# theori-io/nrsc5

Measured on NVIDIA H100. Metric: cu8 I/Q Msamples/s, higher is better.
Workload: dtype u8/int16/f32

## Files before the change

nrsc5_b200/csrc/front.cuh:

```cuda
#pragma once
#include "pids_crc.cuh"
#include "common.cuh"
#include "fft.cuh"
#include "viterbi_pack.cuh"

namespace nb {

constexpr int FRONT_THREADS = 1024;
constexpr int TEAMS = FRONT_THREADS / 128;
constexpr int MAXREF = 15;
constexpr int IN_BYTES = 4 * NSYM + 28 + 16 + 16;
constexpr int IN_STRIDE = 8704;
constexpr int ACQ_TILE = 4096;

__device__ int g_dbg;

__constant__ int c_compat_mode[64];
__constant__ unsigned c_pn80[3];
__constant__ short c_bp_tap[32];

__device__ __forceinline__ float2 cmulf(float2 a, float2 b)
{
    return make_float2(a.x * b.x - a.y * b.y, a.x * b.y + a.y * b.x);
}
__device__ __forceinline__ float2 cexp_j(float a)
{
    float s, c;
    sincosf(a, &s, &c);
    return make_float2(c, s);
}

__device__ __forceinline__ int partitions_per_band(int psmi)
{
    switch (c_compat_mode[psmi & 63]) {
    case 2: return 11;
    case 3: return 12;
    case 5: case 6: case 11: return 14;
    default: return 10;
    }
}

__device__ void set_state(const DevPtrs &p, const EngineDims &d, int s, int ns)
{
    StreamState &st = p.st[s];
    if (st.state == ns) return;
    if (st.state == ST_FINE) log_reserve(p, d, s, REC_LOST_SYNC, 0);
    if (ns == ST_FINE) {
        float fo = (float)(((double)st.prev_angle - 2 * M_PI * st.cfo) * 744187.5 / (2 * M_PI * NFFT));
        uint8_t *w = log_reserve(p, d, s, REC_SYNC, 8);
        if (w) {
            reinterpret_cast<float *>(w)[0] = fo;
            reinterpret_cast<int *>(w)[1] = st.psmi;
        }
    }
    st.state = ns;
}

constexpr int DEMOD_RUN = 17;
constexpr int TEAM_SMEM = IN_STRIDE + NSYM * (int)sizeof(short2);
struct DemodSmem {
    float2 buf[TEAMS][TEAM_SMEM / sizeof(float2)];
    float2 symphase[TEAMS];
};
static_assert(FFT_SMEM_ELEMS * sizeof(float2) <= TEAM_SMEM && TEAM_SMEM % 16 == 0, "a team's FFT buffer");
static_assert(DEMOD_RUN * FFT_THREADS >= NSYM && DEMOD_RUN % 2 == 1, "a symbol's runs");
struct PrepSmem {
    uint32_t words[ACQ_TILE + 40];
    short2 ytile[ACQ_TILE + 32];
    float2 sums[NSYM];
    float red_mag[FRONT_THREADS];
    int red_idx[FRONT_THREADS];
    float2 red_v[FRONT_THREADS];
};
constexpr int ACQ1_RUN = 3;
constexpr int ACQ1_WORDS = (NSYM + 38 + 3 + 3) / 4 * 4;
static_assert(ACQ1_RUN * FRONT_THREADS >= NSYM + 31 && ACQ1_RUN % 2 == 1, "a tile's runs");
struct Acq1Smem {
    uint32_t words[2][ACQ1_WORDS];
    short2 ytile[NSYM + 32];
    float2 ring[2][NSYM];
    float2 sums[NSYM];
    float2 shape[NCP];
    float red_mag[FRONT_THREADS];
    int red_idx[FRONT_THREADS];
    float2 red_v[FRONT_THREADS];
};
struct PidsSmem {
    int8_t vit[PIDS_LEN * 3];
    uint2 dec[PIDS_LEN + 64];
};
constexpr int ZS = 32;
static_assert(2 * MAXREF <= 32, "a reference slot fits the 5 bits of FrontSmem::ref_plan");
constexpr int EQ_LD = BLK + 1;
constexpr int EQ_MAXPART = 12;
constexpr int EQ_ROWS = 2 * EQ_MAXPART * (PW - 1);
struct SyncSmem {
    float phs[BLK][ZS];
    float2 eph[2 * MAXREF][BLK];
    float smag[2 * MAXREF];
    float cfq[2 * MAXREF];
    union {
        float2 eq[EQ_ROWS][EQ_LD];
        struct {
            int offs[76][22];
            int verdict[76];
            int winner;
        } srch;
    };
    float wred[FRONT_THREADS / 32][2];
    float fb_w[2][MAXREF], fb_xy[2][MAXREF + 1];
    float4 rowc[EQ_ROWS];
    int ref_ok[2 * MAXREF], ref_bc[2 * MAXREF], ref_psmi[2 * MAXREF];
    bool px_on[2];
    long long px_T[2];
    uint8_t *soft_w;
    int do_search;
};
struct FrontSmem {
    float2 tw[FFT_TW];
    float2 nco[NSYM];
    float2 zref[BLK][ZS];
    uint8_t ref_plan[128];
    union {
        DemodSmem demod;
        PrepSmem prep;
        Acq1Smem acq1;
        SyncSmem sync;
        PidsSmem pidsq[16];
    } u;
};

__device__ void pids_decode_warp(const DevPtrs &p, const EngineDims &d, int s, int e, PidsSmem &sm, int lane)
{
    const StreamState &st = p.st[s];
    const int bc = st.pids_bc[e];
    const int8_t *pmall = p.pm + (size_t)s * 16 * PM_BLOCK;
    const int8_t PMV[20] = { 10, 2, 18, 6, 14, 8, 16, 0, 12, 4, 11, 3, 19, 7, 15, 9, 17, 1, 13, 5 };
    for (int o = lane; o < PIDS_LEN * 3; o += 32) {
        int8_t v = 0;
        if (o % 6 != 5) {
            unsigned i = (unsigned)bc * 200 + (unsigned)(o - o / 6);
            unsigned part = (unsigned)PMV[i % 20];
            unsigned block = i / 200;
            unsigned k = (i / 20) % 10 + P1_ENC / 320;
            unsigned row = (k * 11) % 32, col = (k * 11 + k / 288) % 36;
            v = pmall[(block * 32 + row) * 720 + part * 36 + col];
        }
        sm.vit[o] = v;
    }
    __syncwarp();
    const int l = lane & 15;
    VitHalf<false> vh;
    vh.init(l);
    vitc_run<false>(vh, sm.vit, PIDS_LEN, PIDS_LEN + 64, 0, PIDS_LEN + 64, 0, sm.dec, lane < 16, l);
    __syncwarp();
    int v = (short)(vh.E & 0xffff), state = 2 * l;
    const int w1 = (short)(vh.O & 0xffff);
    if (w1 > v) { v = w1; state = 2 * l + 1; }
    int v2 = (short)(vh.E >> 16), idx2 = 2 * l + 32;
    const int w3 = (short)(vh.O >> 16);
    if (w3 > v2) { v2 = w3; idx2 = 2 * l + 33; }
    if (v2 > v) { v = v2; state = idx2; }
#pragma unroll
    for (int o = 8; o; o >>= 1) {
        const int ov = __shfl_xor_sync(0xffffffffu, v, o, 16), oi = __shfl_xor_sync(0xffffffffu, state, o, 16);
        if (ov > v || (ov == v && oi < state)) { v = ov; state = oi; }
    }
    if (lane == 0) {
        uint8_t pk[10];
        for (int i = 0; i < 10; i++) pk[i] = 0;
        for (int q = PIDS_LEN + 63; q >= 0; q--) {
            if (q >= 32 && q < 32 + PIDS_LEN) {
                const int i = q - 32;
// ... 4 lines not shown
        }
        if (st.pids_rec[e] != 0xffffffffu) {
            uint8_t *w = p.log + (size_t)s * d.log_cap + st.pids_rec[e];
            for (int i = 0; i < 10; i++) w[i] = pk[i];
            w[10] = (uint8_t)pids_crc12_ok(pk);
        }
    }
}

__device__ void front_pids_flush(const DevPtrs &p, const EngineDims &d, int s, PidsSmem *sm, int t)
{
    StreamState &st = p.st[s];
    const int n = st.pids_pending, warp = t >> 5;
    if (warp < n) pids_decode_warp(p, d, s, warp, sm[warp], t & 31);
    __syncthreads();
    if (t == 0) st.pids_pending = 0;
}

constexpr int ACQ_RUN = 5;
static_assert(ACQ_RUN * FRONT_THREADS >= ACQ_TILE + 31, "a tile's runs");
template <int RUN>
__device__ __forceinline__ void acq_tile_input(const EngineDims &d, const uint32_t *words, short2 *ytile, const StreamState &st,
                                               int i0, int L, int t)
{
    const int kb = i0 == 0 ? 31 : 0;
    if (t < kb) ytile[t] = make_short2(st.bp_hist[t][0], st.bp_hist[t][1]);
    const int n = L + 31 - kb;
    if (d.cs16) {
        for (int k = kb + t; k < L + 31; k += FRONT_THREADS) {
            const uint32_t w = words[k + 7];
            ytile[k] = make_short2((short)(w & 0xffff), (short)(w >> 16));
        }
    } else if (RUN * t < n) {
        const int k = kb + min(RUN * t, n - RUN);
        halfband_run<RUN>(words + k, ytile + k);
    }
}

__device__ __forceinline__ float2 acq_bandpass(const short2 *yy)
{
    short accr = 0, acci = 0;
#pragma unroll 5
    for (int k = 1; k < 16; k++) {
        const short2 a = yy[k], b = yy[32 - k];
        accr = (short)(accr + ((((int)a.x + (int)b.x) * c_bp_tap[k]) >> 15));
        acci = (short)(acci + ((((int)a.y + (int)b.y) * c_bp_tap[k]) >> 15));
    }
    const short2 c = yy[16];
    accr = (short)(accr + (((int)c.x * c_bp_tap[16]) >> 15));
    acci = (short)(acci + (((int)c.y * c_bp_tap[16]) >> 15));
    return make_float2(__fdiv_rn((float)accr, 32767.0f), __fdiv_rn((float)acci, -32767.0f));
}

__device__ __forceinline__ void fill_nco(const DevPtrs &p, float2 *nco, float theta, int t)
{
    for (int j = t; j < NSYM; j += FRONT_THREADS) {
        float2 e = cexp_j(theta * (float)j);
        if (j < NCP || j >= NFFT) {
            const float w = __ldg(&p.shape[j]);
            e = make_float2(e.x * w, e.y * w);
        }
        nco[j] = e;
    }
}

__device__ int front_prep_begin(const DevPtrs &p, const EngineDims &d, int s, int t)
{
    StreamState &st = p.st[s];
    __shared__ int sh_active;
    if (t == 0) {
        if (st.force_state >= 0) {
            set_state(p, d, s, st.force_state);
            st.force_state = -1;
        }
        const long long avail = *reinterpret_cast<volatile long long *>(&st.in_avail);
        int act = avail >= 2 * (st.start + NACQ);
        if (act && st.state == ST_FINE) {
            const int need = px_need_of(c_compat_mode[st.psmi & 63]);
            if (need & ~d.px_enabled) {
                atomicOr(&p.ctl->px_need, (unsigned)need);
                act = 0;
            }
        }
        st.active = act;
        sh_active = act ? (st.state == ST_FINE ? 1 : 2) : 0;
        if (act) atomicAdd(&p.ctl->progress, 1ull);
    }
    __syncthreads();
    const int mode = sh_active;
    __syncthreads();
    return mode;
}

__device__ void front_acq_tiles(const DevPtrs &p, const EngineDims &d, int s, PrepSmem &sm, int t, int rank, int nranks)
{
    StreamState &st = p.st[s];
    const uint8_t *iq = p.iq + (size_t)s * d.in_stride;
    float2 *tb = p.tbuf + (size_t)s * NACQ;
    const long long start = nranks > 1 ? __ldcg(&st.start) : st.start;
    const uint32_t *iqw = reinterpret_cast<const uint32_t *>(iq);
    for (int i0 = rank * ACQ_TILE; i0 < NACQ; i0 += nranks * ACQ_TILE) {
        const int L = min(ACQ_TILE, NACQ - i0);
        const long long w0 = start + i0 - 38;
        for (int v = t; v < L + 38; v += FRONT_THREADS) {
            const long long a = w0 + v;
            sm.words[v] = a >= 0 ? __ldcg(iqw + a) : (d.cs16 ? 0u : 0x7f7f7f7fu);
        }
        __syncthreads();
        acq_tile_input<ACQ_RUN>(d, sm.words, sm.ytile, st, i0, L, t);
        __syncthreads();
        for (int j = t; j < L; j += FRONT_THREADS) tb[i0 + j] = acq_bandpass(sm.ytile + j);
        if (i0 + L == NACQ && t < 31) {
            const short2 v = sm.ytile[L + t];
            st.bp_hist_next[t][0] = v.x;
            st.bp_hist_next[t][1] = v.y;
        }
        __syncthreads();
    }
}

__device__ void front_acq_corr(const DevPtrs &p, int s, int t, int rank, int nranks)
{
    const float2 *tb = p.tbuf + (size_t)s * NACQ;
    float2 *sums = p.acq_sums + (size_t)s * NSYM;
    const int lo = rank * NSYM / nranks, hi = (rank + 1) * NSYM / nranks;
    for (int i = lo + t; i < hi; i += FRONT_THREADS) {
        float2 acc = make_float2(0.f, 0.f);
        for (int j = 0; j < BLK; j++) {
            const float2 a = __ldcg(&tb[i + j * NSYM]), b = __ldcg(&tb[i + j * NSYM + NFFT]);
            float2 pr = cmulf(a, make_float2(b.x, -b.y));
            acc.x += pr.x;
            acc.y += pr.y;
        }
        sums[i] = acc;
    }
}

__device__ void front_prep_finish(const DevPtrs &p, const EngineDims &d, int s, PrepSmem &sm, float2 *nco, int t, int mode)
{
    StreamState &st = p.st[s];
    __shared__ int sh_samperr;
    __shared__ float sh_angle, sh_theta;
    const int state_in = st.state;
    if (mode == 2) {
        const float2 *gs = p.acq_sums + (size_t)s * NSYM;
        for (int i = t; i < NSYM; i += FRONT_THREADS) sm.sums[i] = __ldcg(&gs[i]);
        if (t < 31) {
            st.bp_hist[t][0] = __ldcg(&st.bp_hist_next[t][0]);
            st.bp_hist[t][1] = __ldcg(&st.bp_hist_next[t][1]);
        }
        __syncthreads();
        float best = -1.0f;
        int besti = 0;
        float2 bestv = make_float2(0.f, 0.f);
        for (int i = t; i < NSYM; i += FRONT_THREADS) {
            float2 v = make_float2(0.f, 0.f);
            for (int j = 0; j < NCP; j++) {
                int q = i + j;
                if (q >= NSYM) q -= NSYM;
                const float2 sv = sm.sums[q];
                const float a = __ldg(&p.shape[j]), b = __ldg(&p.shape[j + NFFT]);
                v.x += (sv.x * a) * b;
                v.y += (sv.y * a) * b;
            }
            const float mag = v.x * v.x + v.y * v.y;
            if (mag > best) { best = mag; besti = i; bestv = v; }
        }
        sm.red_mag[t] = best; sm.red_idx[t] = besti; sm.red_v[t] = bestv;
        __syncthreads();
        for (int o = FRONT_THREADS / 2; o; o >>= 1) {
            if (t < o) {
                const float m2 = sm.red_mag[t + o];
                const int i2 = sm.red_idx[t + o];
                if (m2 > sm.red_mag[t] || (m2 == sm.red_mag[t] && i2 < sm.red_idx[t])) {
                    sm.red_mag[t] = m2; sm.red_idx[t] = i2; sm.red_v[t] = sm.red_v[t + o];
                }
            }
            __syncthreads();
        }
        if (t == 0) {
            const float2 w = cmulf(sm.red_v[0], cexp_j(-st.prev_angle));
            const float angle_diff = atan2f(w.y, w.x);
            const float factor = (st.prev_angle != 0.0f) ? 0.25f : 1.0f;
            const float angle = st.prev_angle + (angle_diff * factor);
            st.prev_angle = angle;
            sh_angle = angle;
            sh_samperr = (sm.red_idx[0] + NSYM - 15) % NSYM;
            if (st.state == ST_NONE) st.state = ST_COARSE;
        }
    } else if (t == 0) {
        sh_samperr = NSYM / 2 + st.samperr;
        st.samperr = 0;
        const float angle = st.prev_angle + (-st.angle);
        st.angle = 0;
        st.prev_angle = angle;
        sh_angle = angle;
    }
    __syncthreads();

    const int samperr = sh_samperr;
    const int adj = NSYM / 2 - samperr;
    if (adj != 0) {
        float *cp = p.cphase + (size_t)s * NFFT;
        for (int i = t; i < SIDE; i += FRONT_THREADS) {
            const int bl = LB0 + i, bu = UB1 - i;
            cp[bl] = (float)((double)cp[bl] - (double)(adj * (bl - NFFT / 2) * 2) * M_PI / NFFT);
            cp[bu] = (float)((double)cp[bu] - (double)(adj * (bu - NFFT / 2) * 2) * M_PI / NFFT);
        }
    }
    if (t == 0) {
        float angle = sh_angle;
        angle = (float)((double)angle - 2 * M_PI * st.cfo);
        const float pre = (float)(-adj) * angle / (float)NFFT;
        const float2 ph = cmulf(st.phase, cexp_j(pre));
        const float theta = angle / (float)NFFT;
        st.phase0 = ph;
        st.theta = theta;
        sh_theta = theta;
        st.blk_samperr = samperr;
        st.blk_state_in = state_in;
        double sn, cs;
        sincos((double)theta * (double)(NSYM * BLK), &sn, &cs);
        const float2 pe = cmulf(ph, make_float2((float)cs, (float)sn));
        const float nrm = sqrtf(pe.x * pe.x + pe.y * pe.y);
        st.phase = make_float2(pe.x / nrm, pe.y / nrm);
        uint8_t *w = log_reserve(p, d, s, REC_BLOCK, 32);
        if (w) {
            int *wi = reinterpret_cast<int *>(w);
            float *wf = reinterpret_cast<float *>(w);
            wi[0] = state_in; wi[1] = samperr; wf[2] = angle; wf[3] = ph.x; wf[4] = ph.y; wi[5] = st.cfo;
            wi[6] = (int)(unsigned)(st.start & 0xffffffffLL);
            wi[7] = (int)(st.start >> 32);
        }
    }
    __syncthreads();
    fill_nco(p, nco, sh_theta, t);
    __syncthreads();
}

__device__ bool front_prep_single(const DevPtrs &p, const EngineDims &d, int s, Acq1Smem &sm, float2 *nco, int t)
{
    StreamState &st = p.st[s];
    __shared__ int sh_active, sh_samperr;
    __shared__ float sh_angle, sh_theta;
    if (t == 0) {
        if (st.force_state >= 0) {
            set_state(p, d, s, st.force_state);
            st.force_state = -1;
        }
        const long long avail = *reinterpret_cast<volatile long long *>(&st.in_avail);
        int act = avail >= 2 * (st.start + NACQ);
        if (act && st.state == ST_FINE) {
            const int need = px_need_of(c_compat_mode[st.psmi & 63]);
            if (need & ~d.px_enabled) {
                atomicOr(&p.ctl->px_need, (unsigned)need);
                act = 0;
            }
        }
        st.active = act;
        sh_active = act;
        if (act) atomicAdd(&p.ctl->progress, 1ull);
    }
    __syncthreads();
    if (!sh_active) return false;

    const uint8_t *iq = p.iq + (size_t)s * d.in_stride;
    const int state_in = st.state;
    if (state_in != ST_FINE) {
        const long long start = st.start;
        constexpr int NT = BLK + 1;
        static_assert(NACQ == NT * NSYM, "the window is whole tiles");
        const int woff = (int)((start - 38) & 3);
        static_assert(NSYM % 4 == 0, "tiles start at the same word phase");
        const int nvec = (woff + NSYM + 38 + 3) / 4;
        auto fetch = [&](int T) {
            const long long w0 = start + (long long)T * NSYM - 38;
            const long long w0a = w0 & ~3LL;
            uint4 *dst = reinterpret_cast<uint4 *>(sm.words[T & 1]);
            for (int v = t; v < nvec; v += FRONT_THREADS) {
                const long long a = w0a + 4 * v;
                if (a >= 0) {
#if defined(NB_EMU)
                    dst[v] = *reinterpret_cast<const uint4 *>(iq + 4 * a);
#else
                    asm volatile("cp.async.cg.shared.global [%0], [%1], 16;" ::"r"((unsigned)__cvta_generic_to_shared(dst + v)), "l"(iq + 4 * a) : "memory");
#endif
                } else {
                    const uint32_t z = d.cs16 ? 0u : 0x7f7f7f7fu;
                    dst[v] = make_uint4(z, z, z, z);
                }
            }
#if !defined(NB_EMU)
            asm volatile("cp.async.commit_group;" ::: "memory");
#endif
        };
        for (int i = t; i < NSYM; i += FRONT_THREADS) sm.sums[i] = make_float2(0.f, 0.f);
        if (t < NCP) sm.shape[t] = make_float2(__ldg(&p.shape[t]), __ldg(&p.shape[t + NFFT]));
        fetch(0);
#pragma unroll 1
        for (int T = 0; T <= NT; T++) {
            if (T + 1 < NT) fetch(T + 1);
#if !defined(NB_EMU)
            if (T + 1 < NT) asm volatile("cp.async.wait_group 1;" ::: "memory");
            else asm volatile("cp.async.wait_group 0;" ::: "memory");
#endif
            __syncthreads();
            if (T < NT) acq_tile_input<ACQ1_RUN>(d, sm.words[T & 1] + woff, sm.ytile, st, T * NSYM, NSYM, t);
            if (T >= 2) {
                const float2 *ya = sm.ring[T & 1], *yb = sm.ring[(T - 1) & 1];
                for (int i = t; i < NSYM; i += FRONT_THREADS) {
                    const float2 a = ya[i], b = i + NFFT < NSYM ? ya[i + NFFT] : yb[i + NFFT - NSYM];
                    const float2 pr = cmulf(a, make_float2(b.x, -b.y));
                    sm.sums[i].x += pr.x;
                    sm.sums[i].y += pr.y;
                }
            }
            __syncthreads();
            if (T < NT) {
                float2 *y = sm.ring[T & 1];
                for (int j = t; j < NSYM; j += FRONT_THREADS) y[j] = acq_bandpass(sm.ytile + j);
                if (T == NT - 1 && t < 31) {
                    const short2 v = sm.ytile[NSYM + t];
                    st.bp_hist[t][0] = v.x;
                    st.bp_hist[t][1] = v.y;
                }
            }
        }
        __syncthreads();
        float best = -1.0f;
        int besti = 0;
        float2 bestv = make_float2(0.f, 0.f);
        for (int i = t; i < NSYM; i += FRONT_THREADS) {
            float2 v = make_float2(0.f, 0.f);
            for (int j = 0; j < NCP; j++) {
                int q = i + j;
                if (q >= NSYM) q -= NSYM;
                const float2 sv = sm.sums[q];
                const float2 ab = sm.shape[j];
                v.x += (sv.x * ab.x) * ab.y;
                v.y += (sv.y * ab.x) * ab.y;
            }
            const float mag = v.x * v.x + v.y * v.y;
            if (mag > best) { best = mag; besti = i; bestv = v; }
        }
        sm.red_mag[t] = best; sm.red_idx[t] = besti; sm.red_v[t] = bestv;
        __syncthreads();
        for (int o = FRONT_THREADS / 2; o; o >>= 1) {
            if (t < o) {
                const float m2 = sm.red_mag[t + o];
                const int i2 = sm.red_idx[t + o];
                if (m2 > sm.red_mag[t] || (m2 == sm.red_mag[t] && i2 < sm.red_idx[t])) {
                    sm.red_mag[t] = m2; sm.red_idx[t] = i2; sm.red_v[t] = sm.red_v[t + o];
                }
            }
            __syncthreads();
        }
        if (t == 0) {
            const float2 w = cmulf(sm.red_v[0], cexp_j(-st.prev_angle));
            const float angle_diff = atan2f(w.y, w.x);
            const float factor = (st.prev_angle != 0.0f) ? 0.25f : 1.0f;
            const float angle = st.prev_angle + (angle_diff * factor);
            st.prev_angle = angle;
            sh_angle = angle;
            sh_samperr = (sm.red_idx[0] + NSYM - 15) % NSYM;
            if (st.state == ST_NONE) st.state = ST_COARSE;
        }
    } else if (t == 0) {
        sh_samperr = NSYM / 2 + st.samperr;
        st.samperr = 0;
        const float angle = st.prev_angle + (-st.angle);
        st.angle = 0;
        st.prev_angle = angle;
        sh_angle = angle;
    }
    __syncthreads();

    const int samperr = sh_samperr;
    const int adj = NSYM / 2 - samperr;
    if (adj != 0) {
        float *cp = p.cphase + (size_t)s * NFFT;
        for (int i = t; i < SIDE; i += FRONT_THREADS) {
            const int bl = LB0 + i, bu = UB1 - i;
            cp[bl] = (float)((double)cp[bl] - (double)(adj * (bl - NFFT / 2) * 2) * M_PI / NFFT);
            cp[bu] = (float)((double)cp[bu] - (double)(adj * (bu - NFFT / 2) * 2) * M_PI / NFFT);
        }
    }
    if (t == 0) {
        float angle = sh_angle;
        angle = (float)((double)angle - 2 * M_PI * st.cfo);
        const float pre = (float)(-adj) * angle / (float)NFFT;
        const float2 ph = cmulf(st.phase, cexp_j(pre));
        const float theta = angle / (float)NFFT;
        st.phase0 = ph;
        st.theta = theta;
        sh_theta = theta;
        st.blk_samperr = samperr;
        st.blk_state_in = state_in;
        double sn, cs;
        sincos((double)theta * (double)(NSYM * BLK), &sn, &cs);
        const float2 pe = cmulf(ph, make_float2((float)cs, (float)sn));
        const float nrm = sqrtf(pe.x * pe.x + pe.y * pe.y);
        st.phase = make_float2(pe.x / nrm, pe.y / nrm);
        uint8_t *w = log_reserve(p, d, s, REC_BLOCK, 32);
        if (w) {
            int *wi = reinterpret_cast<int *>(w);
            float *wf = reinterpret_cast<float *>(w);
            wi[0] = state_in; wi[1] = samperr; wf[2] = angle; wf[3] = ph.x; wf[4] = ph.y; wi[5] = st.cfo;
            wi[6] = (int)(unsigned)(st.start & 0xffffffffLL);
            wi[7] = (int)(st.start >> 32);
        }
    }
    __syncthreads();
    fill_nco(p, nco, sh_theta, t);
    __syncthreads();
    return true;
}

__device__ __forceinline__ float2 sample_q15(short2 h)
{
    const float sc = 1.0f / 32767.0f;
    return make_float2((float)h.x * sc, (float)h.y * -sc);
}

__device__ void front_demod(const DevPtrs &p, const EngineDims &d, int s, int sym, DemodSmem &sm, const float2 *nco,
                            const float2 *tw, float2 (*zref)[ZS], const uint8_t *ref_plan,
                            int half, int tl, long long start, int samperr, float theta, float2 phase0)
{
    float2 *buf = sm.buf[half];
    uint8_t *in = reinterpret_cast<uint8_t *>(buf);
    const int bar = 1 + half;
    const long long base = start + samperr + (long long)NSYM * sym;
    const long long b0 = 4 * base - 28;
    const long long b0a = b0 & ~15LL;
    const int off = (int)(b0 - b0a);
    const uint8_t *iq = p.iq + (size_t)s * d.in_stride;
    bar_sync(bar);
    {
        const int nvec = (off + 4 * NSYM + 28 + 15) / 16;
        static_assert(4 * 128 < (4 * NSYM + 28 + 15) / 16 && (12 + 4 * NSYM + 28 + 15) / 16 <= 5 * 128, "a symbol's copies");
        uint4 *dst = reinterpret_cast<uint4 *>(in) + tl;
        const uint8_t *src = iq + b0a + 16 * tl;
        const bool head = b0a < 0;
#pragma unroll
        for (int i = 0; i < 5; i++) {
            if (i == 4 && tl + 4 * 128 >= nvec) break;
            if (!head || b0a + 16 * (tl + 128 * i) >= 0) {
#if defined(NB_EMU)
                dst[128 * i] = *reinterpret_cast<const uint4 *>(src + 2048 * i);
#else
                asm volatile("cp.async.cg.shared.global [%0], [%1], 16;" ::"r"((unsigned)__cvta_generic_to_shared(dst + 128 * i)), "l"(src + 2048 * i) : "memory");
#endif
            } else {
                dst[128 * i] = make_uint4(0x7f7f7f7fu, 0x7f7f7f7fu, 0x7f7f7f7fu, 0x7f7f7f7fu);
            }
        }
#if !defined(NB_EMU)
        asm volatile("cp.async.commit_group;\n\tcp.async.wait_group 0;" ::: "memory");
#endif
    }
    if (tl == 0) {
        double sn, cs;
        sincos((double)theta * (double)(NSYM * sym), &sn, &cs);
        sm.symphase[half] = cmul(phase0, make_float2((float)cs, (float)sn));
    }
    bar_sync(bar);

    const uint32_t *sw = reinterpret_cast<const uint32_t *>(in + off);
    const short2 *y;
    if (d.cs16) {
        y = reinterpret_cast<const short2 *>(sw + 7);
    } else {
        short2 *yw = reinterpret_cast<short2 *>(in + IN_STRIDE);
        const int j0 = min(DEMOD_RUN * tl, NSYM - DEMOD_RUN);
        halfband_run<DEMOD_RUN>(sw + j0, yw + j0);
        y = yw;
        bar_sync(bar);
    }
    float2 v[16];
    v[0] = cmul(sample_q15(y[tl]), nco[tl]);
    if (tl < NCP) {
        const int j = NFFT + tl;
        v[0] = cadd(v[0], cmul(sample_q15(y[j]), nco[j]));
    }
#pragma unroll
    for (int n1 = 1; n1 < 16; n1++) {
        const int j = n1 * 128 + tl;
        v[n1] = cmul(sample_q15(y[j]), nco[j]);
    }
    bar_sync(bar);
    float2 out[2][8];
    fft2048_block<true>(v, out, buf, tw, tl, bar);
    const float2 sp = sm.symphase[half];

    float2 *dst = p.bins + ((size_t)s * BLK + sym) * NBINS;
    const unsigned plan = ref_plan[tl];
    float2 *zp = zref[sym] + (plan & 31u);
    const unsigned pk = plan >> 5;
    auto put = [&](int c, float2 v, unsigned k) {
        dst[c] = v;
        if (pk == k) *zp = v;
    };
#pragma unroll
    for (int h = 0; h < 2; h++) {
        const int q = tl + 128 * h;
        if (q >= 222) put(q - 222, cmul(out[h][5], sp), 4 * h);
        if (q <= 232) put(q + 34, cmul(out[h][6], sp), 4 * h + 1);
        if (q >= 24) put(q + 243, cmul(out[h][1], sp), 4 * h + 2);
        if (q <= 34) put(q + 499, cmul(out[h][2], sp), 4 * h + 3);
    }
}

__device__ __forceinline__ int ref_bin(int slot)
{
    return slot < MAXREF ? LB0 + PW * slot : UB1 - PW * (slot - MAXREF);
}

__device__ __forceinline__ float atan2_short(float y, float x)
{
    const float ax = fabsf(x), ay = fabsf(y);
    const float mx = fmaxf(ax, ay), mn = fminf(ax, ay);
    const float t = mx > 0.f ? __fdividef(mn, mx) : 0.f;
    const float z = t * t;
    float p = 0.0028340641874819994f;
    p = __fmaf_rn(p, z, -0.016005029901862144f);
    p = __fmaf_rn(p, z, 0.042587608098983765f);
    p = __fmaf_rn(p, z, -0.07495445758104324f);
    p = __fmaf_rn(p, z, 0.10636754333972931f);
    p = __fmaf_rn(p, z, -0.14202570915222168f);
    p = __fmaf_rn(p, z, 0.19992484152317047f);
    p = __fmaf_rn(p, z, -0.3333306610584259f);
    p = __fmaf_rn(p, z, 1.0f);
    float r = p * t;
    if (ay > ax) r = 1.57079637f - r;
    if (x < 0.f) r = 3.14159274f - r;
    return copysignf(r, y);
}

__device__ __forceinline__ void costas_row(float2 *z, float *phs, int zs, float &cfreq, float &cphase, int cfo, float alpha, float beta, bool FAST)
{
    const unsigned pat_pos = (1u << 1) | (1u << 5) | (1u << 6) | (1u << 8) | (1u << 21);
    const unsigned pat_neg = (1u << 0) | (1u << 2) | (1u << 3) | (1u << 4) | (1u << 9) | (1u << 13) | (1u << 14) | (1u << 20) |
                             (1u << 22) | (1u << 31);
    const float cfo_freq = (float)(2 * M_PI * cfo * NCP / NFFT);
    const float PI_F = 3.14159274101257324f;
    const float TWO_PI_HI = 6.28318548202514648f, TWO_PI_LO = -1.74845553e-07f;
// ... 34 lines not shown
    }
    cfreq = f;
    cphase = ph;
}

__device__ __forceinline__ int needle_bit(int n, unsigned rsid)
{
    const signed char base[BLK] = { 0, 1, 0, 0, 0, 1, 1, -1, 1, 0, 0, 0, -1, 0, 0, -1,
                                    -1, -1, -1, -1, 0, 1, 0, -1, -1, -1, -1, -1, -1, -1, -1, 0 };
    if (n == 10) return (int)(rsid >> 1);
    if (n == 11) return (int)((rsid >> 1) ^ (rsid & 1));
    return base[n];
}

__device__ int ref_find(const float2 *z, int zs, unsigned rsid)
{
    unsigned raw = 0;
    for (int n = 0; n < BLK; n++)
        if (!(z[n * zs].x <= 0)) raw |= 1u << n;
    for (int pass = 0; pass < 2; pass++) {
        for (int n = 0; n < BLK; n++) {
            int i;
            for (i = 0; i < BLK; i++) {
                const int nb_ = needle_bit(i, rsid);
                if (nb_ < 0) continue;
                if (nb_ != (int)((raw >> ((n + i) & 31)) & 1)) break;
            }
            if (i == BLK) return n;
        }
        raw = ~raw;
    }
    return -1;
}

__device__ __forceinline__ float half_pi_wrap(float a, float b)
{
    float dd = a - b;
    while ((double)dd > M_PI / 2) dd = (float)((double)dd - M_PI);
    while ((double)dd < -M_PI / 2) dd = (float)((double)dd + M_PI);
    return dd;
}

__device__ __forceinline__ int8_t soft_demap(float x, float mult)
{
    const float v = fmaxf(fminf(x, 1.0f), -1.0f) * mult;
    int r = __float2int_rz(v);
    const float f = v - (float)r;
    if (f >= 0.5f) r++;
    else if (f <= -0.5f) r--;
    return (int8_t)r;
}

template <bool CL>
__device__ void front_sync(const DevPtrs &p, const EngineDims &d, int s, SyncSmem &sm, float2 (*zref)[ZS], int t)
{
    StreamState &st = p.st[s];
    float *cfreq = p.cfreq + (size_t)s * NFFT;
    float *cphase = p.cphase + (size_t)s * NFFT;
    float2 *bins = p.bins + (size_t)s * BLK * NBINS;
    auto ldbin = [](const float2 *q) -> float2 { return CL ? __ldcg(q) : *q; };
    const float loop_bw = 0.05f, damping = 0.70710678f;
    const float denom = 1 + (2 * damping * loop_bw) + (loop_bw * loop_bw);
    const float alpha = (4 * damping * loop_bw) / denom, beta = (4 * loop_bw * loop_bw) / denom;

    int ppb = partitions_per_band(st.psmi);
    int nref = ppb + 1;
    long long sy0 = clock64();
    const bool sy_on = st.state == ST_FINE;
    auto sylap = [&](int k) {
        if (t == 0 && sy_on) {
            const long long c1 = clock64();
            st.sy_cyc[k] += (unsigned long long)(c1 - sy0);
            sy0 = c1;
        }
    };
    auto stage_eq = [&](int first, int stride) {
        const int rows = min(ppb, EQ_MAXPART) * (PW - 1), rows2 = 2 * rows;
        const int dn = stride / rows2, dr = stride - dn * rows2;
        int n = first / rows2, r = first - n * rows2;
#pragma unroll 4
        for (; n < BLK;) {
            const int sb = r >= rows, rr = sb ? r - rows : r;
            const int i = rr / (PW - 1);
            const int ci = sb == 0 ? rr + i + 1 : (NBINS - PW) + rr - (2 * PW - 1) * i;
            sm.eq[r][n] = ldbin(&bins[(size_t)n * NBINS + ci]);
            r += dr;
            n += dn;
            if (r >= rows2) { r -= rows2; n++; }
        }
    };
    const bool pre_staged = st.state == ST_FINE && !(g_dbg & 1);
    if (CL) {
        for (int i = t; i < ZS * BLK; i += FRONT_THREADS) {
            const int slot = i & (ZS - 1), n = i / ZS;
            const int ii = slot < MAXREF ? slot : slot - MAXREF;
            if (slot < 2 * MAXREF && ii < nref) zref[n][slot] = ldbin(&bins[(size_t)n * NBINS + compact_of_bin(ref_bin(slot))]);
        }
        __syncthreads();
    }
    sylap(0);
    if (t < 2 * MAXREF) {
        const int i = t < MAXREF ? t : t - MAXREF;
        if (i < nref) {
            const int b = ref_bin(t);
            float f = cfreq[b], ph = cphase[b];
            costas_row(&zref[0][t], &sm.phs[0][t], ZS, f, ph, 0, alpha, beta, !(g_dbg & 2));
            cfreq[b] = f;
// ... 261 lines not shown
                const int per_sym = nq * 36;
                for (int item = td; item < BLK * nq * 9; item += DSTRIDE) {
                    const int n = item / (nq * 9), rem = item - n * (nq * 9);
                    const int q = rem / 9, c4 = rem - q * 9;
                    const int sb = q >= nq / 2;
                    const int i = nq == 2 ? base : ((q == 0 || q == 3) ? base : base + 1);
                    float2 a, b;
                    if (i < eqparts) {
                        const int r = (sb ? rows : 0) + i * (PW - 1) + 2 * c4;
                        a = sm.eq[r][n];
                        b = sm.eq[r + 1][n];
                    } else {
                        const int ci = (sb == 0 ? PW * i : (NBINS - 1 - PW) - PW * i) + 1 + 2 * c4;
                        a = ldbin(&bins[(size_t)n * NBINS + ci]);
                        b = ldbin(&bins[(size_t)n * NBINS + ci + 1]);
                    }
                    const float ml = mult[lower_scale_only ? 0 : sb];
                    const unsigned w = (unsigned)(uint8_t)soft_demap(a.x, ml) | ((unsigned)(uint8_t)soft_demap(a.y, ml) << 8) |
                                       ((unsigned)(uint8_t)soft_demap(b.x, ml) << 16) | ((unsigned)(uint8_t)soft_demap(b.y, ml) << 24);
                    const long long pos = (T + n * per_sym + q * 36 + 4 * c4) % PX_RING;
                    *reinterpret_cast<uint32_t *>(ring + pos) = w;
                }
            };
            if (sm.px_on[0]) px_demap(p.px_ring[0] + (size_t)s * PX_RING, sm.px_T[0], cm == 2 ? 2 : 4, 10, false);
            if (sm.px_on[1]) px_demap(p.px_ring[1] + (size_t)s * PX_RING, sm.px_T[1], 4, 12, true);
        } else if (t >= 32) {
            const int lane = t & 31;
            if (lane < ppb) {
                sm.fb_w[0][lane] = half_pi_wrap(sm.phs[0][lane], sm.phs[0][lane + 1]);
                sm.fb_w[1][lane] = half_pi_wrap(sm.phs[0][MAXREF + lane + 1], sm.phs[0][MAXREF + lane]);
            }
            if (lane <= ppb) {
                sm.fb_xy[0][lane] = (float)(LB0 + PW * lane - NFFT / 2) * sm.cfq[lane];
                sm.fb_xy[1][lane] = (float)(UB1 - PW * lane - NFFT / 2) * sm.cfq[MAXREF + lane];
            }
            __syncwarp();
            float fb_angle = 0;
            if (lane == 31) {
                float samperr = 0, angle = 0, sum_xy = 0, sum_x2 = 0;
                for (int i = 0; i < ppb; i++) {
                    samperr += sm.fb_w[0][i];
                    samperr += sm.fb_w[1][i];
                }
                const double inv_2pi = 1.0 / (2 * M_PI);
                samperr = (float)((double)(samperr / (float)(ppb * 2) * (float)NFFT / (float)PW) * inv_2pi);
                for (int i = 0; i <= ppb; i++) {
                    float x;
                    x = (float)(LB0 + PW * i - NFFT / 2);
                    angle += sm.cfq[i]; sum_xy += sm.fb_xy[0][i]; sum_x2 += x * x;
                    x = (float)(UB1 - PW * i - NFFT / 2);
                    angle += sm.cfq[MAXREF + i]; sum_xy += sm.fb_xy[1][i]; sum_x2 += x * x;
                }
                samperr = (float)((double)samperr - (double)((sum_xy / sum_x2) * (float)NFFT) * inv_2pi * BLK);
                st.samperr = (int)roundf(samperr);
                angle /= (float)((ppb + 1) * 2);
                st.angle = angle;
                fb_angle = angle;
            }
            fb_angle = __shfl_sync(0xffffffffu, fb_angle, 31);
            const int i = lane < MAXREF ? lane : lane - MAXREF;
            if (lane < 2 * MAXREF && i < nref) cfreq[ref_bin(lane)] = sm.cfq[lane] - fb_angle;
        } else if (t == 0) {
            st.err_lb += e_sb[0];
            st.err_ub += e_sb[1];
            if (++st.mer_cnt == 16) {
                const float signal = (float)(2 * BLK * (ppb * 18) * st.mer_cnt);
                uint8_t *w = log_reserve(p, d, s, REC_MER, 8);
                if (w) {
                    reinterpret_cast<float *>(w)[0] = 10 * log10f(signal / st.err_lb);
                    reinterpret_cast<float *>(w)[1] = 10 * log10f(signal / st.err_ub);
                }
                st.mer_cnt = 0;
                st.err_lb = 0;
                st.err_ub = 0;
            }
            if (d.emit_soft) {
                sm.soft_w = log_reserve(p, d, s, REC_SOFT_PM, 4 + PM_BLOCK);
                if (sm.soft_w) *reinterpret_cast<uint32_t *>(sm.soft_w) = (uint32_t)bc;
            }
            uint8_t *w = log_reserve(p, d, s, REC_PIDS, 11);
            const int e = st.pids_pending;
            st.pids_rec[e] = w ? (unsigned)(w - (p.log + (size_t)s * d.log_cap)) : 0xffffffffu;
            st.pids_bc[e] = bc;
            st.pids_pending = e + 1;
            if (bc == 0) st.started_pm = 1;
            unsigned lost_slot = 0xffffffffu;
            if (st.started_pm && bc == 15) {
                const unsigned len0 = st.log_len;
                uint8_t *bw = log_reserve(p, d, s, REC_BER, 4);
                uint8_t *fw = bw ? log_reserve(p, d, s, REC_FRAME, 8 + P1_LEN / 8) : nullptr;
                if (!fw) { st.log_len = len0; bw = nullptr; }
                st.p1_rec = (bw && fw) ? (unsigned)(bw - (p.log + (size_t)s * d.log_cap)) : 0xffffffffu;
                if (fw) {
                    reinterpret_cast<uint32_t *>(fw)[0] = 0;
                    reinterpret_cast<uint32_t *>(fw)[1] = P1_LEN;
                    uint8_t *lw = log_reserve(p, d, s, REC_PAD, 0);
                    if (lw) lost_slot = (unsigned)(lw - 8 - (p.log + (size_t)s * d.log_cap));
                }
                st.p1_lost_rec = lost_slot;
                l2_enqueue(st, d.l2, st.p1_rec != 0xffffffffu ? st.p1_rec + 4 + 8 + 8 : 0xffffffffu, 0, P1_LEN);
                st.p1_ready = 1;
            }
#pragma unroll
            for (int g = 0; g < PX_GROUPS; g++) {
                const PxGroup x = px_group(g);
                if (!(x.modes >> cm & 1)) continue;
                if ((bc & 1) == 0) st.px_started[x.ring] = 1;
                if (!st.px_started[x.ring]) continue;
                st.px_total[x.ring] += x.len;
                const long long k0 = st.px_total[x.ring] - 2 * x.len;
// ... 15 lines not shown
                st.p1_lost_rec = 0xffffffffu;
            }
            st.bc = (bc + 1) % 16;
        }
        __syncthreads();
        if (d.emit_soft && sm.soft_w)
            for (int o = t; o < PM_BLOCK; o += FRONT_THREADS) sm.soft_w[4 + o] = (uint8_t)pm[o];
    }
    if (t == 0) {
        const int keep = NSYM + (NSYM / 2 - st.blk_samperr) + st.keep_extra;
        st.keep_extra = 0;
        st.start += NACQ - keep;
        st.blocks_done++;
    }
    sylap(5);
}

__device__ __forceinline__ void cluster_barrier()
{
#if defined(NB_EMU)
#else
    asm volatile("barrier.cluster.arrive.release.aligned;\n\tbarrier.cluster.wait.acquire.aligned;" ::: "memory");
#endif
}

template <bool CL>
__global__ void __launch_bounds__(FRONT_THREADS, 1) k_stream(DevPtrs p, EngineDims d, int max_blocks, int last_pass)
{
#if defined(NB_EMU)
    unsigned char *front_smem_raw = emu::dyn_smem();
#else
    extern __shared__ __align__(16) unsigned char front_smem_raw[];
#endif
    FrontSmem &sm = *reinterpret_cast<FrontSmem *>(front_smem_raw);
    const int t = threadIdx.x, team = t >> 7, tl = t & 127;
    const int C = CL ? d.cluster : 1;
    const int s = (int)blockIdx.x / C, rank = (int)blockIdx.x % C;
    StreamState &st = p.st[s];
    for (int i = t; i < FFT_TW; i += FRONT_THREADS) sm.tw[i] = __ldg(&p.twid[i]);
    if (t < 128) {
        unsigned m = 0xffu;
        for (int h = 0; h < 2; h++) {
            const int q = t + 128 * h;
            const int c[4] = { q >= 222 ? q - 222 : -1, q <= 232 ? q + 34 : -1, q >= 24 ? q + 243 : -1, q <= 34 ? q + 499 : -1 };
            for (int k = 0; k < 4; k++) {
                if (c[k] < 0) continue;
                const int slot = c[k] < SIDE ? (c[k] % PW == 0 ? c[k] / PW : -1)
                                             : ((NBINS - 1 - c[k]) % PW == 0 ? MAXREF + (NBINS - 1 - c[k]) / PW : -1);
                if (slot >= 0) m = (unsigned)(4 * h + k) << 5 | (unsigned)slot;
            }
        }
        sm.ref_plan[t] = (uint8_t)m;
    }
    __syncthreads();

    const bool owner = !CL || rank == 0;
    if (max_blocks > 16) max_blocks = 16;
    if (owner && t == 0) {
        for (int g = 0; g < PX_GROUPS; g++) st.xq_pending[g] = 0;
    }
    __syncthreads();
    for (int nb = 0;; nb++) {
        long long c0 = clock64();
        auto lap = [&](int ph) {
            if (owner && t == 0) {
                const long long c1 = clock64();
                st.ph_cyc[ph] += (unsigned long long)(c1 - c0);
                st.ph_n[ph]++;
                c0 = c1;
            }
        };
        int mode = 0;
        if (!CL) {
            if (nb < max_blocks && !st.p1_ready) mode = front_prep_single(p, d, s, sm.u.acq1, sm.nco, t) ? 1 : 0;
            if (mode == 0) break;
        } else {
            if (owner) {
                if (nb < max_blocks && !st.p1_ready) mode = front_prep_begin(p, d, s, t);
                if (mode == 1) front_prep_finish(p, d, s, sm.u.prep, sm.nco, t, 1);
            }
            if (owner && t == 0) {
                st.blk_go = mode;
                __threadfence();
            }
            cluster_barrier();
            if (!owner) mode = __ldcg(&st.blk_go);
            if (mode == 0) break;
            if (mode == 2) {
                front_acq_tiles(p, d, s, sm.u.prep, t, rank, C);
                __threadfence();
                cluster_barrier();
                front_acq_corr(p, s, t, rank, C);
                __threadfence();
                cluster_barrier();
                if (owner) {
                    front_prep_finish(p, d, s, sm.u.prep, sm.nco, t, 2);
                    __threadfence();
                }
                cluster_barrier();
            }
        }
        lap(st.blk_state_in == ST_FINE ? 2 : 1);
        const long long start = CL ? __ldcg(&st.start) : st.start;
        const int samperr = CL ? __ldcg(&st.blk_samperr) : st.blk_samperr;
        const float theta = CL ? __ldcg(&st.theta) : st.theta;
        const float2 phase0 = CL ? __ldcg(&st.phase0) : st.phase0;
        if (CL && !owner) {
            fill_nco(p, sm.nco, theta, t);
            __syncthreads();
        }
#pragma unroll 1
        for (int pass = 0; pass < BLK / (TEAMS * C); pass++)
            front_demod(p, d, s, (pass * C + rank) * TEAMS + team, sm.u.demod, sm.nco, sm.tw, sm.zref, sm.ref_plan, team, tl, start, samperr, theta, phase0);
        if (CL) {
            __threadfence();
            cluster_barrier();
        }
        if (CL && !owner) continue;
        __syncthreads();
        lap(3);
        front_sync<CL>(p, d, s, sm.u.sync, sm.zref, t);
        __syncthreads();
        lap(st.blk_state_in == ST_FINE ? 4 : 5);
    }
    if (CL && !owner) return;
    __syncthreads();
    if (st.pids_pending) {
        const long long c0 = clock64();
        front_pids_flush(p, d, s, sm.u.pidsq, t);
        if (t == 0) {
            st.ph_cyc[0] += (unsigned long long)(clock64() - c0);
            st.ph_n[0]++;
        }
    }
    if (t == 0) {
        StreamBrief b;
        b.start = st.start;
        b.state = st.state;
        b.bc = st.bc;
        b.p1_ready = st.p1_ready;
        b.pad_ = 0;
        p.brief[s] = b;
        const long long avail = *reinterpret_cast<volatile long long *>(&st.in_avail);
        if (last_pass && avail >= 2 * (st.start + NACQ)) atomicAdd(&p.ctl->more, 1u);
    }
}

}
```

Baseline: 172,700.

## Precompute next block's NCO and symbol phases during sync, overlap with prep

In the non-cluster path, the sync stage now computes the next block's samperr, angle, theta and phase0 into a shared BlockSet. The following prep call can then fill the NCO and per-symbol phase tables on threads 1..N-1 while thread 0 runs the availability and state checks. It also skips the redundant prep-finish sequence in FINE state. Per-symbol phase sincos moves out of each demod team into a shared table filled once per block, which removes a serial double-precision sincos from the demod critical path. The speculative NCO fill depends on b.ok bookkeeping staying consistent with stream state changes such as force_state.

```diff
diff --git a/nrsc5_b200/csrc/front.cuh b/nrsc5_b200/csrc/front.cuh
--- a/nrsc5_b200/csrc/front.cuh
+++ b/nrsc5_b200/csrc/front.cuh
@@ -60,7 +60,6 @@
 constexpr int TEAM_SMEM = IN_STRIDE + NSYM * (int)sizeof(short2);
 struct DemodSmem {
     float2 buf[TEAMS][TEAM_SMEM / sizeof(float2)];
-    float2 symphase[TEAMS];
 };
 static_assert(FFT_SMEM_ELEMS * sizeof(float2) <= TEAM_SMEM && TEAM_SMEM % 16 == 0, "a team's FFT buffer");
 static_assert(DEMOD_RUN * FFT_THREADS >= NSYM && DEMOD_RUN % 2 == 1, "a symbol's runs");
@@ -116,9 +115,18 @@
     uint8_t *soft_w;
     int do_search;
 };
+struct BlockSet {
+    int samperr;
+    int ok;
+    float prev_angle, angle;
+    float theta;
+    float2 phase0, phase;
+};
 struct FrontSmem {
     float2 tw[FFT_TW];
     float2 nco[NSYM];
+    float2 symphase[BLK];
+    BlockSet blk;
     float2 zref[BLK][ZS];
     uint8_t ref_plan[128];
     union {
@@ -229,15 +237,69 @@
     return make_float2(__fdiv_rn((float)accr, 32767.0f), __fdiv_rn((float)acci, -32767.0f));
 }
 
-__device__ __forceinline__ void fill_nco(const DevPtrs &p, float2 *nco, float theta, int t)
-{
-    for (int j = t; j < NSYM; j += FRONT_THREADS) {
+__device__ __forceinline__ void fill_nco(const DevPtrs &p, float2 *nco, float theta, int t, int nthreads = FRONT_THREADS)
+{
+    for (int j = t; j < NSYM; j += nthreads) {
         float2 e = cexp_j(theta * (float)j);
         if (j < NCP || j >= NFFT) {
             const float w = __ldg(&p.shape[j]);
             e = make_float2(e.x * w, e.y * w);
         }
         nco[j] = e;
+    }
+}
+
+__device__ __forceinline__ void fill_symphase(float2 *symphase, float theta, float2 phase0, int sym)
+{
+    double sn, cs;
+    sincos((double)theta * (double)(NSYM * sym), &sn, &cs);
+    symphase[sym] = cmul(phase0, make_float2((float)cs, (float)sn));
+}
+
+__device__ __forceinline__ void block_setup(BlockSet &b, const StreamState &st)
+{
+    const int adj = NSYM / 2 - b.samperr;
+    float angle = b.prev_angle;
+    angle = (float)((double)angle - 2 * M_PI * st.cfo);
+    const float pre = (float)(-adj) * angle / (float)NFFT;
+    const float2 ph = cmulf(st.phase, cexp_j(pre));
+    const float theta = angle / (float)NFFT;
+    double sn, cs;
+    sincos((double)theta * (double)(NSYM * BLK), &sn, &cs);
+    const float2 pe = cmulf(ph, make_float2((float)cs, (float)sn));
+    const float nrm = sqrtf(pe.x * pe.x + pe.y * pe.y);
+    b.angle = angle;
+    b.theta = theta;
+    b.phase0 = ph;
+    b.phase = make_float2(pe.x / nrm, pe.y / nrm);
+}
+
+__device__ __forceinline__ void sync_adjust(const DevPtrs &p, int s, int adj, int t)
+{
+    if (adj == 0) return;
+    float *cp = p.cphase + (size_t)s * NFFT;
+    for (int i = t; i < SIDE; i += FRONT_THREADS) {
+        const int bl = LB0 + i, bu = UB1 - i;
+        cp[bl] = (float)((double)cp[bl] - (double)(adj * (bl - NFFT / 2) * 2) * M_PI / NFFT);
+        cp[bu] = (float)((double)cp[bu] - (double)(adj * (bu - NFFT / 2) * 2) * M_PI / NFFT);
+    }
+}
+
+__device__ __forceinline__ void block_commit(const DevPtrs &p, const EngineDims &d, int s, const BlockSet &b, int state_in)
+{
+    StreamState &st = p.st[s];
+    st.phase0 = b.phase0;
+    st.theta = b.theta;
+    st.blk_samperr = b.samperr;
+    st.blk_state_in = state_in;
+    st.phase = b.phase;
+    uint8_t *w = log_reserve(p, d, s, REC_BLOCK, 32);
+    if (w) {
+        int *wi = reinterpret_cast<int *>(w);
+        float *wf = reinterpret_cast<float *>(w);
+        wi[0] = state_in; wi[1] = b.samperr; wf[2] = b.angle; wf[3] = b.phase0.x; wf[4] = b.phase0.y; wi[5] = st.cfo;
+        wi[6] = (int)(unsigned)(st.start & 0xffffffffLL);
+        wi[7] = (int)(st.start >> 32);
     }
 }
 
@@ -313,11 +375,10 @@
     }
 }
 
-__device__ void front_prep_finish(const DevPtrs &p, const EngineDims &d, int s, PrepSmem &sm, float2 *nco, int t, int mode)
+__device__ void front_prep_finish(const DevPtrs &p, const EngineDims &d, int s, PrepSmem &sm, float2 *nco, float2 *symphase,
+                                  BlockSet &b, int t, int mode)
 {
     StreamState &st = p.st[s];
-    __shared__ int sh_samperr;
-    __shared__ float sh_angle, sh_theta;
     const int state_in = st.state;
     if (mode == 2) {
         const float2 *gs = p.acq_sums + (size_t)s * NSYM;
@@ -361,85 +422,74 @@
             const float factor = (st.prev_angle != 0.0f) ? 0.25f : 1.0f;
             const float angle = st.prev_angle + (angle_diff * factor);
             st.prev_angle = angle;
-            sh_angle = angle;
-            sh_samperr = (sm.red_idx[0] + NSYM - 15) % NSYM;
+            b.prev_angle = angle;
+            b.samperr = (sm.red_idx[0] + NSYM - 15) % NSYM;
             if (st.state == ST_NONE) st.state = ST_COARSE;
         }
     } else if (t == 0) {
-        sh_samperr = NSYM / 2 + st.samperr;
+        b.samperr = NSYM / 2 + st.samperr;
         st.samperr = 0;
         const float angle = st.prev_angle + (-st.angle);
         st.angle = 0;
         st.prev_angle = angle;
-        sh_angle = angle;
+        b.prev_angle = angle;
     }
     __syncthreads();
-
-    const int samperr = sh_samperr;
-    const int adj = NSYM / 2 - samperr;
-    if (adj != 0) {
-        float *cp = p.cphase + (size_t)s * NFFT;
-        for (int i = t; i < SIDE; i += FRONT_THREADS) {
-            const int bl = LB0 + i, bu = UB1 - i;
-            cp[bl] = (float)((double)cp[bl] - (double)(adj * (bl - NFFT / 2) * 2) * M_PI / NFFT);
-            cp[bu] = (float)((double)cp[bu] - (double)(adj * (bu - NFFT / 2) * 2) * M_PI / NFFT);
-        }
-    }
+    sync_adjust(p, s, NSYM / 2 - b.samperr, t);
     if (t == 0) {
-        float angle = sh_angle;
-        angle = (float)((double)angle - 2 * M_PI * st.cfo);
-        const float pre = (float)(-adj) * angle / (float)NFFT;
-        const float2 ph = cmulf(st.phase, cexp_j(pre));
-        const float theta = angle / (float)NFFT;
-        st.phase0 = ph;
-        st.theta = theta;
-        sh_theta = theta;
-        st.blk_samperr = samperr;
-        st.blk_state_in = state_in;
-        double sn, cs;
-        sincos((double)theta * (double)(NSYM * BLK), &sn, &cs);
-        const float2 pe = cmulf(ph, make_float2((float)cs, (float)sn));
-        const float nrm = sqrtf(pe.x * pe.x + pe.y * pe.y);
-        st.phase = make_float2(pe.x / nrm, pe.y / nrm);
-        uint8_t *w = log_reserve(p, d, s, REC_BLOCK, 32);
-        if (w) {
-            int *wi = reinterpret_cast<int *>(w);
-            float *wf = reinterpret_cast<float *>(w);
-            wi[0] = state_in; wi[1] = samperr; wf[2] = angle; wf[3] = ph.x; wf[4] = ph.y; wi[5] = st.cfo;
-            wi[6] = (int)(unsigned)(st.start & 0xffffffffLL);
-            wi[7] = (int)(st.start >> 32);
-        }
+        block_setup(b, st);
+        block_commit(p, d, s, b, state_in);
     }
     __syncthreads();
-    fill_nco(p, nco, sh_theta, t);
+    fill_nco(p, nco, b.theta, t);
+    if (t >= FRONT_THREADS - BLK) fill_symphase(symphase, b.theta, b.phase0, t - (FRONT_THREADS - BLK));
     __syncthreads();
 }
 
-__device__ bool front_prep_single(const DevPtrs &p, const EngineDims &d, int s, Acq1Smem &sm, float2 *nco, int t)
+__device__ bool front_prep_single(const DevPtrs &p, const EngineDims &d, int s, Acq1Smem &sm, float2 *nco, float2 *symphase,
+                                  BlockSet &b, int t)
 {
     StreamState &st = p.st[s];
-    __shared__ int sh_active, sh_samperr;
-    __shared__ float sh_angle, sh_theta;
+    __shared__ int sh_active;
     if (t == 0) {
-        if (st.force_state >= 0) {
-            set_state(p, d, s, st.force_state);
+        const int fs = st.force_state;
+        const long long avail = *reinterpret_cast<volatile long long *>(&st.in_avail);
+        const long long start = st.start;
+        const int psmi = st.psmi;
+        int state = st.state;
+        if (fs >= 0) {
+            set_state(p, d, s, fs);
             st.force_state = -1;
-        }
-        const long long avail = *reinterpret_cast<volatile long long *>(&st.in_avail);
-        int act = avail >= 2 * (st.start + NACQ);
-        if (act && st.state == ST_FINE) {
-            const int need = px_need_of(c_compat_mode[st.psmi & 63]);
+            state = fs;
+        }
+        int act = avail >= 2 * (start + NACQ);
+        if (act && state == ST_FINE) {
+            const int need = px_need_of(c_compat_mode[psmi & 63]);
             if (need & ~d.px_enabled) {
                 atomicOr(&p.ctl->px_need, (unsigned)need);
                 act = 0;
             }
         }
         st.active = act;
-        sh_active = act;
+        sh_active = act ? (state == ST_FINE && b.ok ? 2 : 1) : 0;
+        b.ok = 0;
         if (act) atomicAdd(&p.ctl->progress, 1ull);
+    } else {
+        fill_nco(p, nco, b.theta, t - 1, FRONT_THREADS - 1);
+        if (t >= FRONT_THREADS - BLK) fill_symphase(symphase, b.theta, b.phase0, t - (FRONT_THREADS - BLK));
     }
     __syncthreads();
     if (!sh_active) return false;
+    if (sh_active == 2) {
+        sync_adjust(p, s, NSYM / 2 - b.samperr, t);
+        if (t == 0) {
+            st.samperr = 0;
+            st.angle = 0;
+            st.prev_angle = b.prev_angle;
+            block_commit(p, d, s, b, ST_FINE);
+        }
+        return true;
+    }
 
     const uint8_t *iq = p.iq + (size_t)s * d.in_stride;
     const int state_in = st.state;
@@ -538,57 +588,27 @@
             const float factor = (st.prev_angle != 0.0f) ? 0.25f : 1.0f;
             const float angle = st.prev_angle + (angle_diff * factor);
             st.prev_angle = angle;
-            sh_angle = angle;
-            sh_samperr = (sm.red_idx[0] + NSYM - 15) % NSYM;
+            b.prev_angle = angle;
+            b.samperr = (sm.red_idx[0] + NSYM - 15) % NSYM;
             if (st.state == ST_NONE) st.state = ST_COARSE;
         }
     } else if (t == 0) {
-        sh_samperr = NSYM / 2 + st.samperr;
+        b.samperr = NSYM / 2 + st.samperr;
         st.samperr = 0;
         const float angle = st.prev_angle + (-st.angle);
         st.angle = 0;
         st.prev_angle = angle;
-        sh_angle = angle;
+        b.prev_angle = angle;
     }
     __syncthreads();
-
-    const int samperr = sh_samperr;
-    const int adj = NSYM / 2 - samperr;
-    if (adj != 0) {
-        float *cp = p.cphase + (size_t)s * NFFT;
-        for (int i = t; i < SIDE; i += FRONT_THREADS) {
-            const int bl = LB0 + i, bu = UB1 - i;
-            cp[bl] = (float)((double)cp[bl] - (double)(adj * (bl - NFFT / 2) * 2) * M_PI / NFFT);
-            cp[bu] = (float)((double)cp[bu] - (double)(adj * (bu - NFFT / 2) * 2) * M_PI / NFFT);
-        }
-    }
+    sync_adjust(p, s, NSYM / 2 - b.samperr, t);
     if (t == 0) {
-        float angle = sh_angle;
-        angle = (float)((double)angle - 2 * M_PI * st.cfo);
-        const float pre = (float)(-adj) * angle / (float)NFFT;
-        const float2 ph = cmulf(st.phase, cexp_j(pre));
-        const float theta = angle / (float)NFFT;
-        st.phase0 = ph;
-        st.theta = theta;
-        sh_theta = theta;
-        st.blk_samperr = samperr;
-        st.blk_state_in = state_in;
-        double sn, cs;
-        sincos((double)theta * (double)(NSYM * BLK), &sn, &cs);
-        const float2 pe = cmulf(ph, make_float2((float)cs, (float)sn));
-        const float nrm = sqrtf(pe.x * pe.x + pe.y * pe.y);
-        st.phase = make_float2(pe.x / nrm, pe.y / nrm);
-        uint8_t *w = log_reserve(p, d, s, REC_BLOCK, 32);
-        if (w) {
-            int *wi = reinterpret_cast<int *>(w);
-            float *wf = reinterpret_cast<float *>(w);
-            wi[0] = state_in; wi[1] = samperr; wf[2] = angle; wf[3] = ph.x; wf[4] = ph.y; wi[5] = st.cfo;
-            wi[6] = (int)(unsigned)(st.start & 0xffffffffLL);
-            wi[7] = (int)(st.start >> 32);
-        }
+        block_setup(b, st);
+        block_commit(p, d, s, b, state_in);
     }
     __syncthreads();
-    fill_nco(p, nco, sh_theta, t);
+    fill_nco(p, nco, b.theta, t);
+    if (t >= FRONT_THREADS - BLK) fill_symphase(symphase, b.theta, b.phase0, t - (FRONT_THREADS - BLK));
     __syncthreads();
     return true;
 }
@@ -600,8 +620,8 @@
 }
 
 __device__ void front_demod(const DevPtrs &p, const EngineDims &d, int s, int sym, DemodSmem &sm, const float2 *nco,
-                            const float2 *tw, float2 (*zref)[ZS], const uint8_t *ref_plan,
-                            int half, int tl, long long start, int samperr, float theta, float2 phase0)
+                            const float2 *symphase, const float2 *tw, float2 (*zref)[ZS], const uint8_t *ref_plan,
+                            int half, int tl, long long start, int samperr)
 {
     float2 *buf = sm.buf[half];
     uint8_t *in = reinterpret_cast<uint8_t *>(buf);
@@ -635,11 +655,6 @@
         asm volatile("cp.async.commit_group;\n\tcp.async.wait_group 0;" ::: "memory");
 #endif
     }
-    if (tl == 0) {
-        double sn, cs;
-        sincos((double)theta * (double)(NSYM * sym), &sn, &cs);
-        sm.symphase[half] = cmul(phase0, make_float2((float)cs, (float)sn));
-    }
     bar_sync(bar);
 
     const uint32_t *sw = reinterpret_cast<const uint32_t *>(in + off);
@@ -667,7 +682,7 @@
     bar_sync(bar);
     float2 out[2][8];
     fft2048_block<true>(v, out, buf, tw, tl, bar);
-    const float2 sp = sm.symphase[half];
+    const float2 sp = symphase[sym];
 
     float2 *dst = p.bins + ((size_t)s * BLK + sym) * NBINS;
     const unsigned plan = ref_plan[tl];
@@ -808,7 +823,7 @@
 }
 
 template <bool CL>
-__device__ void front_sync(const DevPtrs &p, const EngineDims &d, int s, SyncSmem &sm, float2 (*zref)[ZS], int t)
+__device__ void front_sync(const DevPtrs &p, const EngineDims &d, int s, SyncSmem &sm, float2 (*zref)[ZS], BlockSet &b, int t)
 {
     StreamState &st = p.st[s];
     float *cfreq = p.cfreq + (size_t)s * NFFT;
@@ -1176,10 +1191,17 @@
                     angle += sm.cfq[MAXREF + i]; sum_xy += sm.fb_xy[1][i]; sum_x2 += x * x;
                 }
                 samperr = (float)((double)samperr - (double)((sum_xy / sum_x2) * (float)NFFT) * inv_2pi * BLK);
-                st.samperr = (int)roundf(samperr);
+                const int se = (int)roundf(samperr);
+                st.samperr = se;
                 angle /= (float)((ppb + 1) * 2);
                 st.angle = angle;
                 fb_angle = angle;
+                if (!CL) {
+                    b.samperr = NSYM / 2 + se;
+                    b.prev_angle = st.prev_angle + (-angle);
+                    block_setup(b, st);
+                    b.ok = 1;
+                }
             }
             fb_angle = __shfl_sync(0xffffffffu, fb_angle, 31);
             const int i = lane < MAXREF ? lane : lane - MAXREF;
@@ -1301,6 +1323,11 @@
         }
         sm.ref_plan[t] = (uint8_t)m;
     }
+    if (t == 0) {
+        sm.blk.ok = 0;
+        sm.blk.theta = 0.f;
+        sm.blk.phase0 = make_float2(0.f, 0.f);
+    }
     __syncthreads();
 
     const bool owner = !CL || rank == 0;
@@ -1321,12 +1348,12 @@
         };
         int mode = 0;
         if (!CL) {
-            if (nb < max_blocks && !st.p1_ready) mode = front_prep_single(p, d, s, sm.u.acq1, sm.nco, t) ? 1 : 0;
+            if (nb < max_blocks && !st.p1_ready) mode = front_prep_single(p, d, s, sm.u.acq1, sm.nco, sm.symphase, sm.blk, t) ? 1 : 0;
             if (mode == 0) break;
         } else {
             if (owner) {
                 if (nb < max_blocks && !st.p1_ready) mode = front_prep_begin(p, d, s, t);
-                if (mode == 1) front_prep_finish(p, d, s, sm.u.prep, sm.nco, t, 1);
+                if (mode == 1) front_prep_finish(p, d, s, sm.u.prep, sm.nco, sm.symphase, sm.blk, t, 1);
             }
             if (owner && t == 0) {
                 st.blk_go = mode;
@@ -1343,7 +1370,7 @@
                 __threadfence();
                 cluster_barrier();
                 if (owner) {
-                    front_prep_finish(p, d, s, sm.u.prep, sm.nco, t, 2);
+                    front_prep_finish(p, d, s, sm.u.prep, sm.nco, sm.symphase, sm.blk, t, 2);
                     __threadfence();
                 }
                 cluster_barrier();
@@ -1351,16 +1378,17 @@
         }
         lap(st.blk_state_in == ST_FINE ? 2 : 1);
         const long long start = CL ? __ldcg(&st.start) : st.start;
-        const int samperr = CL ? __ldcg(&st.blk_samperr) : st.blk_samperr;
-        const float theta = CL ? __ldcg(&st.theta) : st.theta;
-        const float2 phase0 = CL ? __ldcg(&st.phase0) : st.phase0;
+        const int samperr = CL ? __ldcg(&st.blk_samperr) : sm.blk.samperr;
         if (CL && !owner) {
+            const float theta = __ldcg(&st.theta);
             fill_nco(p, sm.nco, theta, t);
+            if (t >= FRONT_THREADS - BLK) fill_symphase(sm.symphase, theta, __ldcg(&st.phase0), t - (FRONT_THREADS - BLK));
             __syncthreads();
         }
 #pragma unroll 1
         for (int pass = 0; pass < BLK / (TEAMS * C); pass++)
-            front_demod(p, d, s, (pass * C + rank) * TEAMS + team, sm.u.demod, sm.nco, sm.tw, sm.zref, sm.ref_plan, team, tl, start, samperr, theta, phase0);
+            front_demod(p, d, s, (pass * C + rank) * TEAMS + team, sm.u.demod, sm.nco, sm.symphase, sm.tw, sm.zref, sm.ref_plan,
+                            team, tl, start, samperr);
         if (CL) {
             __threadfence();
             cluster_barrier();
@@ -1368,7 +1396,7 @@
         if (CL && !owner) continue;
         __syncthreads();
         lap(3);
-        front_sync<CL>(p, d, s, sm.u.sync, sm.zref, t);
+        front_sync<CL>(p, d, s, sm.u.sync, sm.zref, sm.blk, t);
         __syncthreads();
         lap(st.blk_state_in == ST_FINE ? 4 : 5);
     }
```

Measured after the change: 180,600 (median of 6 runs). 1.05x the previous value.
